# QWTforGithub/CDSegNet

Measured on AMD Instinct MI355X. Metric: points/sec/node (ScanNet ~120k-pt scenes, 1-step), higher is better.
Workload: dtype f16

## Files before the change

### cdsegnet_amd/_lib.py

```python
import ctypes
import os
import threading
from ctypes import POINTER, Structure, c_char_p, c_float, c_int, c_int32, c_int64, c_long, c_size_t, c_uint64, c_void_p

HERE = os.path.dirname(os.path.abspath(__file__))
LIB_PATH = os.path.join(HERE, "libcdseg_hip.so")
LIB_PATH_F16 = os.path.join(HERE, "libcdseg_hip_f16.so")

F32, BF16 = 0, 1
ACT_NONE, ACT_GELU, ACT_SWISH = 0, 1, 2
ORDER_IDS = {"z": 0, "z-trans": 1, "hilbert": 2, "hilbert-trans": 3}
ERRORS = {-1: "CDSEG_ERR_ARG", -2: "CDSEG_ERR_LAUNCH", -3: "CDSEG_ERR_WORKSPACE", -4: "CDSEG_ERR_UNSUPPORTED"}


class CdsegError(RuntimeError):
    pass


class DuplicateVoxelsError(CdsegError):

    def __init__(self, msg, count):
        super().__init__(msg)
        self.count = int(count)

# ... 126 lines not shown
    "cdseg_attn_tail_fused": (c_int, [c_void_p, c_int, c_void_p, c_void_p, c_void_p, c_void_p, c_float, c_void_p, c_void_p,
                                      c_void_p, c_void_p, c_void_p, c_int, c_void_p, c_int, c_long, c_int, c_int, c_void_p]),
    "cdseg_cpe_head_fused": (c_int, [c_void_p, c_int, c_void_p, c_void_p, c_void_p, c_void_p, c_void_p, c_int, c_void_p,
                                     c_void_p, c_void_p, c_float, c_void_p, c_void_p, c_void_p, c_int, c_long, c_int, c_int,
                                     c_int, c_void_p]),
    "cdseg_subm_conv3_wimg_bytes": (c_size_t, [c_int]),
    "cdseg_subm_conv3_pack": (c_int, [c_void_p, c_int, c_void_p, c_void_p]),
    "cdseg_subm_conv3": (c_int, [c_void_p, c_int, c_void_p, c_void_p, c_void_p, c_long, c_int, c_void_p, c_int, c_void_p]),
    "cdseg_child_info": (c_int, [c_void_p, c_void_p, c_long, c_void_p, c_void_p]),
    "cdseg_stem5_wimg_bytes": (c_size_t, []),
    "cdseg_stem5_pack": (c_int, [c_void_p, c_void_p, c_void_p]),
    "cdseg_stem5": (c_int, [c_void_p, c_void_p, c_void_p, c_void_p, c_void_p, c_void_p, c_void_p, c_void_p, c_long, c_long,
                            c_int, c_void_p, c_void_p, c_void_p]),
    "cdseg_block_rr_img_bytes": (c_size_t, [c_int, c_int]),
    "cdseg_block_rr_pack": (c_int, [c_int, c_void_p, c_void_p, c_void_p, c_void_p, c_void_p, c_void_p, c_void_p, c_void_p]),
    "cdseg_cpe_head_rr": (c_int, [c_void_p, c_int, c_void_p, c_void_p, c_void_p, c_void_p, c_void_p, c_int, c_void_p, c_void_p,
                                  c_void_p, c_float, c_void_p, c_void_p, c_int, c_long, c_int, c_int, c_void_p]),
    "cdseg_attn_tail_rr": (c_int, [c_void_p, c_int, c_void_p, c_void_p, c_void_p, c_void_p, c_float, c_void_p, c_void_p,
                                   c_void_p, c_int, c_void_p, c_int, c_long, c_int, c_void_p]),
    "cdseg_cpe_head_rr2": (c_int, [c_void_p, c_int, c_void_p, c_void_p, c_void_p, c_void_p, c_void_p, c_int, c_void_p, c_int,
                                   c_void_p, c_void_p, c_void_p, c_float, c_void_p, c_void_p, c_int, c_long, c_int, c_int, c_void_p]),
    "cdseg_attn_tail_rr2": (c_int, [c_void_p, c_int, c_void_p, c_void_p, c_void_p, c_void_p, c_float, c_void_p, c_void_p,
                                    c_void_p, c_int, c_void_p, c_int, c_void_p, c_int, c_long, c_int, c_void_p, c_size_t, c_void_p]),
    "cdseg_block_scratch_bytes": (c_size_t, [POINTER(BlockDesc), c_long]),
    "cdseg_block_forward": (c_int, [POINTER(BlockDesc), POINTER(BlockIO), c_void_p]),
    "cdseg_layernorm": (c_int, [c_void_p, c_int, c_int, c_void_p, c_void_p, c_float, c_void_p, c_int, c_void_p,
                                c_void_p, c_int, c_int, c_void_p, c_int, c_int, c_long, c_int, c_void_p]),
    "cdseg_attention": (c_int, [c_void_p, c_void_p, c_void_p, c_int, c_int, c_int, c_void_p, c_void_p, c_void_p,
                                c_void_p, c_int, c_int, c_int, c_float, c_void_p, c_int, c_int, c_void_p]),
    "cdseg_attention_ex": (c_int, [c_void_p, c_void_p, c_void_p, c_int, c_int, c_int, c_void_p, c_void_p, c_void_p,
                                   c_void_p, c_int, c_int, c_int, c_float, c_void_p, c_int, c_int, c_int, c_void_p]),
    "cdseg_attention_schedule": (c_long, [c_int, c_int, c_int, c_int, c_void_p, c_long]),
    "cdseg_attention_bwd_ws_bytes": (c_size_t, [c_long, c_int]),
    "cdseg_attention_bwd": (c_int, [c_void_p, c_void_p, c_void_p, c_int, c_int, c_int, c_void_p, c_void_p, c_void_p, c_void_p,
                                    c_int, c_int, c_long, c_int, c_float, c_void_p, c_int, c_void_p, c_void_p, c_void_p,
                                    c_int, c_int, c_int, c_int, c_void_p, c_size_t, c_void_p]),
    "cdseg_layernorm_bwd": (c_int, [c_void_p, c_int, c_void_p, c_float, c_void_p, c_int, c_void_p, c_int, c_int, c_void_p,
                                    c_void_p, c_long, c_int, c_void_p]),
    "cdseg_gelu_bwd": (c_int, [c_void_p, c_void_p, c_void_p, c_long, c_void_p]),
    "cdseg_conv_wgrad": (c_int, [c_void_p, c_int, c_void_p, c_int, c_void_p, c_int, c_long, c_int, c_int, c_void_p, c_void_p,
                                 c_void_p]),
    "cdseg_linear_wgrad": (c_int, [c_void_p, c_int, c_void_p, c_void_p, c_int, c_long, c_int, c_int, c_void_p, c_int, c_void_p,
                                   c_void_p]),
    "cdseg_prof_enable": (c_int, [c_int]),
    "cdseg_prof_summary": (c_int, [POINTER(ctypes.c_double), POINTER(c_long)]),
    "cdseg_prof_summary_class": (c_int, [c_int, POINTER(ctypes.c_double), POINTER(c_long)]),
    "cdseg_segment_max": (c_int, [c_void_p, c_int, c_int, c_void_p, c_long, c_int, c_void_p, c_void_p, c_int,
                                  c_void_p, c_int, c_void_p, c_int, c_int, c_void_p]),
    "cdseg_segment_mean": (c_int, [c_void_p, c_int, c_void_p, c_long, c_int, c_void_p, c_int, c_void_p]),
    "cdseg_pool_fused_img_bytes": (c_size_t, [c_int, c_int]),
    "cdseg_pool_fused_pack": (c_int, [c_void_p, c_int, c_int, c_void_p, c_void_p]),
    "cdseg_pool_fused": (c_int, [c_void_p, c_int, c_void_p, c_void_p, c_void_p, c_long, c_void_p, c_void_p, c_int, c_void_p, c_int,
                                 c_void_p, c_int, c_int, c_int, c_void_p]),
    "cdseg_gemv": (c_int, [c_void_p, c_void_p, c_void_p, c_int, c_int, c_int, c_void_p, c_void_p]),
    "cdseg_randn": (c_int, [c_void_p, c_long, c_uint64, c_uint64, c_void_p]),
    "cdseg_cast": (c_int, [c_void_p, c_int, c_void_p, c_int, c_long, c_void_p]),
    "cdseg_gather_pad_cast": (c_int, [c_void_p, c_int, c_void_p, c_long, c_int, c_int, c_void_p, c_int, c_void_p]),
    "cdseg_ddim_update": (c_int, [c_void_p, c_void_p, c_float, c_float, c_float, c_float, c_int, c_void_p, c_long,
                                  c_void_p]),
    "cdseg_axpy": (c_int, [c_void_p, c_void_p, c_float, c_void_p, c_long, c_void_p]),
    "cdseg_count_saturated": (c_int, [c_void_p, c_long, c_int, c_int, c_void_p, c_void_p]),
    "cdseg_subm_conv3_f32": (c_int, [c_void_p, c_int, c_void_p, c_void_p, c_void_p, c_long, c_int, c_void_p, c_int, c_float, c_int,
                                     c_void_p]),
    "cdseg_split16": (c_int, [c_void_p, c_int, c_long, c_int, c_void_p, c_void_p, c_int, c_float, c_void_p]),
}

_libs = {}
_tls = threading.local()
VARIANTS = ("bf16", "f16")


def active():
    return getattr(_tls, "variant", "bf16")


class use:

    def __init__(self, variant):
        if variant not in VARIANTS:
            raise ValueError(variant)
        self.variant = variant

    def __enter__(self):
        self.prev = active()
        _tls.variant = self.variant
        return self

    def __exit__(self, *exc):
        _tls.variant = self.prev
        return False


def activate(variant):
    if variant not in VARIANTS:
        raise ValueError(variant)
    _tls.variant = variant


def load(variant=None):
    v = variant or active()
    lib = _libs.get(v)
    if lib is not None:
        return lib
    path = LIB_PATH if v == "bf16" else LIB_PATH_F16
    if not os.path.exists(path):
        raise CdsegError(
# ... 15 lines not shown
```

### cdsegnet_amd/csrc/pool.hip

```cpp
#include <atomic>

#include "common.h"

namespace {

struct PoolP {
  const bf16_t* x; const uint4* wimg; const float* bias; const int32_t* seg; const float* scale; const float* shift;
  float* out; bf16_t* out2;
  long m;
  int ldx, ldo, ldo2, act;
};

constexpr int PL_WAVES = 8;

template <int CIN, int COUT>
struct PoolCfg {
  static constexpr int KS = CIN / 32, OT = COUT / 16, QI = CIN / 4, QO = COUT / 4;
  static constexpr int W_BYTES = CIN * COUT * 2;
  static constexpr int ROW = COUT * 2 + 16;
  static constexpr int STRIP = 16 * ROW;
  static constexpr int PAR = 3 * COUT * 4;
  static constexpr int LDS = W_BYTES + PL_WAVES * STRIP + PAR;
};

// ... 102 lines not shown
      float* o = p.out + mrow * p.ldo + q * QO;
#pragma unroll
      for (int c4 = 0; c4 < QO / 4; ++c4) {
        const f32x4_t sc = *reinterpret_cast<const f32x4_t*>(pr + COUT + q * QO + 4 * c4);
        const f32x4_t sh = *reinterpret_cast<const f32x4_t*>(pr + 2 * COUT + q * QO + 4 * c4);
        f32x4_t v;
#pragma unroll
        for (int r = 0; r < 4; ++r) {
          v[r] = __builtin_fmaf(mx[4 * c4 + r], sc[r], sh[r]);
          if (p.act == CDSEG_ACT_GELU) v[r] = gelu_erf(v[r]);
        }
        *reinterpret_cast<f32x4_t*>(o + 4 * c4) = v;
        if (p.out2) {
          uint2 u;
          u.x = pack_bf16x2(v[0], v[1]);
          u.y = pack_bf16x2(v[2], v[3]);
          *reinterpret_cast<uint2*>(p.out2 + mrow * p.ldo2 + q * QO + 4 * c4) = u;
        }
      }
    }
  }
}

__global__ void pool_pack_kernel(const bf16_t* __restrict__ w, uint4* __restrict__ img, int cin, int cout) {
  const int KS = cin / 32;
  const int u = blockIdx.x * blockDim.x + threadIdx.x;
  if (u >= (cout / 16) * KS * 64) return;
  const int lane = u & 63, s = (u >> 6) % KS, ot = (u >> 6) / KS;
  const int q = lane >> 4, i = lane & 15;
  const long row = (i >> 2) * (cout / 4) + ot * 4 + (i & 3);
  img[u] = *reinterpret_cast<const uint4*>(w + row * cin + 32 * s + 8 * q);
}

template <int CIN, int COUT>
int launch_pool(const PoolP& p, hipStream_t s) {
  using K = PoolCfg<CIN, COUT>;
  static std::atomic<bool> attr_done{false};
  if (!attr_done) {
    if (hipFuncSetAttribute((const void*)pool_fused_kernel<CIN, COUT>, hipFuncAttributeMaxDynamicSharedMemorySize, K::LDS) != hipSuccess)
      return CDSEG_ERR_LAUNCH;
    attr_done = true;
  }
  const long chunks = (p.m + 15) / 16;
  long blocks = (chunks + PL_WAVES - 1) / PL_WAVES;
  const int per_cu = K::LDS > 80 * 1024 ? 1 : (K::LDS > 52 * 1024 ? 2 : 3);
  if (blocks > 256 * per_cu) blocks = 256 * per_cu;
  hipLaunchKernelGGL((pool_fused_kernel<CIN, COUT>), dim3((unsigned)blocks), dim3(PL_WAVES * 64), K::LDS, s, p);
  CDSEG_CHECK_LAUNCH();
  return CDSEG_OK;
}

bool pool_supported(int cin, int cout) { return (cin == 32 && cout == 64) || (cin == 64 && cout == 128); }

}

extern "C" size_t cdseg_pool_fused_img_bytes(int cin, int cout) { return pool_supported(cin, cout) ? (size_t)cin * cout * 2 : 0; }

extern "C" int cdseg_pool_fused_pack(const void* w, int cin, int cout, void* wimg, void* stream) {
  if (!w || !wimg || (((uintptr_t)w | (uintptr_t)wimg) & 15)) return CDSEG_ERR_ARG;
  if (!pool_supported(cin, cout)) return CDSEG_ERR_UNSUPPORTED;
  const int units = (cout / 16) * (cin / 32) * 64;
  hipLaunchKernelGGL(pool_pack_kernel, dim3((units + 255) / 256), dim3(256), 0, (hipStream_t)stream, (const bf16_t*)w, (uint4*)wimg, cin,
                     cout);
  CDSEG_CHECK_LAUNCH();
  return CDSEG_OK;
}

extern "C" int cdseg_pool_fused(const void* x, int ldx, const void* wimg, const float* bias, const int32_t* seg_start, long m,
                                const float* scale, const float* shift, int act, float* out, int ldo, void* out2, int ldo2,
                                int cin, int cout, void* stream) {
  if (m <= 0) return CDSEG_OK;
  if (!x || !wimg || !seg_start || !out) return CDSEG_ERR_ARG;
  if (!pool_supported(cin, cout) || (act != CDSEG_ACT_NONE && act != CDSEG_ACT_GELU)) return CDSEG_ERR_UNSUPPORTED;
  if ((ldx & 7) || (ldo & 3) || (out2 && (ldo2 & 3)) || (((uintptr_t)x | (uintptr_t)wimg | (uintptr_t)out) & 15) ||
      (out2 && (((uintptr_t)out2) & 7)) || (bias && (((uintptr_t)bias) & 15)) || (scale && (((uintptr_t)scale) & 15)) ||
      (shift && (((uintptr_t)shift) & 15)) || (!scale != !shift))
    return CDSEG_ERR_ARG;
  PoolP p;
  p.x = (const bf16_t*)x; p.wimg = (const uint4*)wimg; p.bias = bias; p.seg = seg_start; p.scale = scale; p.shift = shift;
  p.out = out; p.out2 = (bf16_t*)out2; p.m = m; p.ldx = ldx; p.ldo = ldo; p.ldo2 = ldo2; p.act = act;
  hipStream_t s = (hipStream_t)stream;
  if (cin == 32) return launch_pool<32, 64>(p, s);
  return launch_pool<64, 128>(p, s);
}
```

### cdsegnet_amd/engine.py

```python
import math
import struct
import os
import threading

import numpy as np
import torch

from . import _lib, ops
from ._lib import CdsegError, DuplicateVoxelsError

CURVES = ("z", "z-trans", "hilbert", "hilbert-trans")


def _pooling_depth(stride):
    return (math.ceil(stride) - 1).bit_length()


class _ShareEvents(threading.local):
    on = False


SHARE_EVENTS = _ShareEvents()


# ... 291 lines not shown

        def bn(mod, pre):
            scale = mod.weight.detach().double() / torch.sqrt(mod.running_var.detach().double() + mod.eps)
            shift = mod.bias.detach().double() - mod.running_mean.detach().double() * scale
            w[pre + ".scale"], w[pre + ".shift"] = f32(scale), f32(shift)

        self.block_desc = {}

        def block(mod, pre):
            self._blocks_to_describe.append((mod, pre))
            conv(mod.cpe[0], pre + ".cpe0")
            lin(mod.cpe[1], pre + ".cpe1")
            ln(mod.cpe[2], pre + ".cpe2")
            ln(mod.norm1[0], pre + ".norm1")
            lin_q(mod.attn.qkv, pre + ".qkv", mod.attn.scale, mod.channels)
            lin(mod.attn.proj, pre + ".proj")
            ln(mod.norm2[0], pre + ".norm2")
            lin(mod.mlp[0].fc1, pre + ".fc1")
            lin(mod.mlp[0].fc2, pre + ".fc2")

        def stem(mod, pre):
            cw = mod.stem.conv.weight.detach()
            cout, cin = cw.shape[0], cw.shape[-1]
            cpad = (cin + 7) // 8 * 8
            wp = torch.zeros(cout, cw.shape[1] ** 3, cpad, dtype=torch.float32)
            wp[:, :, :cin] = cw.reshape(cout, -1, cin).float().cpu()
            w[pre + ".w"] = wp.reshape(cout, -1).to(device=device, dtype=T).contiguous()
            w[pre + ".cpad"] = cpad
            if cw.shape[1] == 5 and cpad == 8 and hasattr(ops, "stem5_pack") and ops.stem5_ok(cout, T):
                w[pre + ".wimg"] = ops.stem5_pack(w[pre + ".w"])
            bn(mod.stem.norm, pre + ".bn")

        def pool(mod, pre):
            lin(mod.proj, pre + ".proj")
            bn(mod.norm[0], pre + ".bn")
            pw = w[pre + ".proj.w"]
            if hasattr(ops, "pool_fused_ok") and ops.pool_fused_ok(pw.shape[1], pw.shape[0], T):
                w[pre + ".proj.wimg"] = ops.pool_fused_pack(pw)

        def unpool(mod, pre):
            lin(mod.proj[0], pre + ".proj")
            bn(mod.proj[1], pre + ".proj_bn")
            lin(mod.proj_skip[0], pre + ".skip")
            bn(mod.proj_skip[1], pre + ".skip_bn")
            if mod.skip_connection_mode == "cat":
                f = (2 ** -0.5 if mod.skip_connection_scale else 1.0)
                if mod.skip_connection_scale_i is not None:
                    f *= 0.8 ** (int(mod.skip_connection_scale_i) - 1)
                wc = mod.proj_cat[0].weight.detach().float()
                c = wc.shape[0]
                w[pre + ".cat_a.w"] = (wc[:, :c] * f).to(device=device, dtype=T).contiguous()
                w[pre + ".cat_b.w"] = wc[:, c:].to(device=device, dtype=T).contiguous()
                w[pre + ".cat.b"] = f32(mod.proj_cat[0].bias)

        bb = self.model.backbone
        stem(bb._n_embedding, "n_emb")
        for s in range(bb.n_num_stages):
            enc = getattr(bb._n_enc, f"enc{s}")
            if s > 0:
                pool(enc.down, f"n_enc{s}.down")
            for name, mod in enc._modules.items():
                if name.startswith("block"):
                    block(mod, f"n_enc{s}.{name}")
        for s in range(bb.n_num_stages - 1):
            dec = getattr(bb._n_dec, f"dec{s}")
            unpool(dec.up, f"n_dec{s}.up")
            for name, mod in dec._modules.items():
                if name.startswith("block"):
                    block(mod, f"n_dec{s}.{name}")
        if isinstance(bb._n_head, torch.nn.Linear):
            lin(bb._n_head, "n_head")
        if bb.condition:
            stem(bb._c_embedding, "c_emb")
            tw, tb, toff = [], [], {}
            off = 0
            for s in range(bb.c_num_stages):
                enc = getattr(bb._c_enc, f"enc{s}")
                if s > 0:
                    pool(enc.down, f"c_enc{s}.down")
                for name, mod in enc._modules.items():
                    if name.startswith("block"):
                        block(mod, f"c_enc{s}.{name}")
                        if bb.T_dim != -1:
                            tw.append(f32(mod.t_mlp.weight))
                            tb.append(f32(mod.t_mlp.bias))
                            toff[f"c_enc{s}.{name}"] = (off, off + mod.channels)
                            off += mod.channels
            for s in range(bb.c_num_stages - 1):
                dec = getattr(bb._c_dec, f"dec{s}")
                unpool(dec.up, f"c_dec{s}.up")
                for name, mod in dec._modules.items():
                    if name.startswith("block"):
                        block(mod, f"c_dec{s}.{name}")
                        if bb.T_dim != -1:
                            tw.append(f32(mod.t_mlp.weight))
                            tb.append(f32(mod.t_mlp.bias))
                            toff[f"c_dec{s}.{name}"] = (off, off + mod.channels)
                            off += mod.channels
            if isinstance(bb._c_head, torch.nn.Linear):
                lin(bb._c_head, "c_head")
            if bb.T_dim != -1:
                w["t.fc1.w"], w["t.fc1.b"] = f32(bb.fc_t1.weight), f32(bb.fc_t1.bias)
                w["t.fc2.w"], w["t.fc2.b"] = f32(bb.fc_t2.weight), f32(bb.fc_t2.bias)
                w["t.mlp.w"], w["t.mlp.b"] = torch.cat(tw).contiguous(), torch.cat(tb).contiguous()
                w["t.table"] = f32(self.model.t_emb_table)
                self.t_slices = toff
# ... 578 lines not shown
            ops.gemm(o, w[pre + ".proj.w"], st.x, bias=w[pre + ".proj.b"], res=st.x)
        self._mlp(st, pre + ".norm2", pre + ".fc", h2)

    def run_embedding(self, plan, feat, perm, pre, curves):
        w, lv = self.w, plan.levels[0]
        cout = w[pre + ".w"].shape[0]
        a = ops.gather_pad_cast(feat, perm, w[pre + ".cpad"], self.T)
        x = self._buf(lv.n, cout, torch.float32)
        xc = x if self.T == torch.float32 else self._buf(lv.n, cout, self.T)
        if (pre + ".wimg") in w and lv.parent is not None and lv.n < (1 << 24):
            par, (cluster, seg) = lv.parent
            ops.stem5(a, w[pre + ".wimg"], w[pre + ".bn.scale"], w[pre + ".bn.shift"], lv.grid, cluster, par.nbr(3, True),
                      lv.child_info(), lv.depth, x, None if xc is x else xc)
        else:
            ops.gemm(a, w[pre + ".w"], x, scale=w[pre + ".bn.scale"], shift=w[pre + ".bn.shift"], act=ops.ACT_GELU,
                     nbr=lv.nbr(5, True), nbr_kmajor=True, kvol=125, out2=None if xc is x else xc)
        self._sat_note(xc)
        return State(lv, x, xc, curves)

    def run_pooling(self, plan, st, pre, cum_to, perm):
        w = self.w
        fine, coarse = st.level, plan.levels[cum_to]
        _, seg = plan.link(fine.cum, cum_to)
        cout = w[pre + ".proj.w"].shape[0]
        x = self._buf(coarse.n, cout, torch.float32)
        xc = x if self.T == torch.float32 else self._buf(coarse.n, cout, self.T)
        if (pre + ".proj.wimg") in w and st.xc.stride(0) == st.xc.shape[1] and fine.n <= 5 * coarse.n:
            ops.pool_fused(st.xc, w[pre + ".proj.wimg"], w[pre + ".proj.b"], seg, coarse.n, w[pre + ".bn.scale"],
                           w[pre + ".bn.shift"], ops.ACT_GELU, x, xc)
        else:
            y = self._buf(fine.n, cout, self.T)
            ops.gemm(st.xc, w[pre + ".proj.w"], y, bias=w[pre + ".proj.b"])
            ops.segment_max(y, seg, coarse.n, w[pre + ".bn.scale"], w[pre + ".bn.shift"], ops.ACT_GELU, x,
                            None if xc is x else xc)
        self._sat_note(xc)
        curves = st.curves if perm is None else [st.curves[int(j)] for j in perm]
        out = State(coarse, x, xc, curves)
        out.parent = st
        return out

    def run_unpooling(self, plan, st, pre, mod):
        w = self.w
        parent = st.parent
        fine, coarse = parent.level, st.level
        cluster, _ = plan.link(fine.cum, coarse.cum)
        cout = w[pre + ".proj.w"].shape[0]
        f = (2 ** -0.5 if mod.skip_connection_scale else 1.0)
        if mod.skip_connection_scale_i is not None:
            f *= 0.8 ** (int(mod.skip_connection_scale_i) - 1)
        x = self._buf(fine.n, cout, torch.float32)
        xc = self._buf(fine.n, cout, self.T)
        if mod.skip_connection_mode == "add":
            assert f == 1.0, "rejected by SerializedUnpooling.__init__"
            child = self._buf(coarse.n, cout, torch.float32)
            ops.gemm(st.xc, w[pre + ".proj.w"], child, bias=w[pre + ".proj.b"], scale=w[pre + ".proj_bn.scale"],
                     shift=w[pre + ".proj_bn.shift"], act=ops.ACT_GELU)
            ops.gemm(parent.xc, w[pre + ".skip.w"], x, bias=w[pre + ".skip.b"], scale=w[pre + ".skip_bn.scale"],
                     shift=w[pre + ".skip_bn.shift"], act=ops.ACT_GELU, add_src=child, add_idx=cluster, out2=xc,
                     out2_pre_add=True)
        else:
            child = self._buf(coarse.n, cout, self.T)
            ops.gemm(st.xc, w[pre + ".proj.w"], child, bias=w[pre + ".proj.b"], scale=w[pre + ".proj_bn.scale"],
                     shift=w[pre + ".proj_bn.shift"], act=ops.ACT_GELU)
            z = self._buf(coarse.n, cout, torch.float32)
            ops.gemm(child, w[pre + ".cat_b.w"], z)
            ops.gemm(parent.xc, w[pre + ".skip.w"], xc, bias=w[pre + ".skip.b"], scale=w[pre + ".skip_bn.scale"],
                     shift=w[pre + ".skip_bn.shift"], act=ops.ACT_GELU)
            ops.gemm(xc, w[pre + ".cat_a.w"], x, bias=w[pre + ".cat.b"], add_src=z, add_idx=cluster)
        self._sat_note(xc)
        out = State(fine, x, xc, parent.curves)
        out.parent = parent.parent
        return out

    def run_cross_block(self, nst, cst):
        w = self.w
        cb = self.model.backbone._tm_dec0.cross_block2
        att = cb.attn
        lv, clv = nst.level, cst.level
        if clv is not lv and list(clv.offs_host) != list(lv.offs_host):
            raise CdsegError("cross attention needs the same number of c- and n-branch bottleneck points per batch "
                             "element (ref: ptv3.py:1009 reuses the q padding for kv)")
        n, cq = nst.x.shape
        self._cpe(nst, "x.q_cpe", nst.xc)
        self._cpe(cst, "x.kv_cpe", cst.xc)
        hq = self._buf(n, cq, self.T)
        ops.layernorm(nst.x, w["x.q_norm1.g"], w["x.q_norm1.b"], hq)
        hkv = self._buf(n, cst.x.shape[1], self.T)
        ops.layernorm(cst.x, w["x.kv_norm1.g"], w["x.kv_norm1.b"], hkv)
        cst.xc = hkv
        if self.T == torch.float32:
            cst.x = hkv
        q = self._buf(n, cq, self.T)
        ops.gemm(hq, w["x.q.w"], q, bias=w["x.q.b"])
        kv = self._buf(n, 2 * cq, self.T)
        ops.gemm(hkv, w["x.kv.w"], kv, bias=w["x.kv.b"])
        K = att.q_patch_size
        q_gidx, widx = lv.slots(nst.curves[att.order_index], K, att.enable_flash)
        kv_gidx, _ = clv.slots(cst.curves[att.order_index], K, att.enable_flash)
        _, _, _, _, patch_start, max_len, sum_l2 = lv.pad(K, att.enable_flash)
        work = 64.0 * att.num_heads * lv.attn_l2(K, att.enable_flash)
        self._add_work(work, 4.0 * n * cq * q.element_size())
        o = self._buf(n, cq, self.T)
        ops.attention(q, kv[:, :cq], kv[:, cq:], q_gidx, kv_gidx, widx, patch_start, att.num_heads, max_len, att.scale, o,
                      work=work, flags=ops.ATTN_Q_PRESCALED if self.q_prescaled else 0)
        if "x.tail_img" in w and n >= ops.DEEP512_MIN_ROWS:
            nst.xc = self._buf(n, cq, self.T)
            ops.attn_tail_rr(o, w["x.tail_img"], w["x.proj.b"], w["x.q_norm2.g"], w["x.q_norm2.b"], w["x.fc1.b"], w["x.fc2.b"],
                             nst.x, nst.xc)
            return
        if "x.tail_img" in w and hasattr(ops, "attn_tail_rr2"):
            x_new = self._buf(n, cq, torch.float32)
            nst.xc = self._buf(n, cq, self.T)
# ... 356 lines not shown
```

### cdsegnet_amd/ops.py

```python
import ctypes
import os
import threading

import torch

from . import _lib
from ._lib import ACT_GELU, ACT_NONE, ACT_SWISH, BF16, F32, GemmArgs, check

__all__ = ["ACT_NONE", "ACT_GELU", "ACT_SWISH", "F32", "BF16"]

LP_DTYPES = {"bf16": torch.bfloat16, "f16": torch.float16}


class _Dtypes:

    def __getitem__(self, dtype):
        if dtype == torch.float32:
            return F32
        if dtype == LP_DTYPES[_lib.active()]:
            return BF16
        raise _lib.CdsegError(f"{dtype} tensors do not belong to the active build of the library ({_lib.active()})")


_DT = _Dtypes()
# ... 743 lines not shown
                                      out2.stride(0) if out2 is not None else 0, m, c, _stream()), "layernorm")
    return out


ATTN_Q_PRESCALED, ATTN_V_BF16 = 1, 2


def attention(q, k, v, q_gidx, kv_gidx, widx, patch_start, num_heads, max_len, scale, out, work=0.0, flags=0):
    num_patches = patch_start.numel() - 1
    if not (q.dtype == k.dtype == out.dtype) or (v.dtype != q.dtype and not (flags & ATTN_V_BF16)):
        raise _lib.CdsegError("attention: q, k, v, out must share a dtype")
    tok = TIMER.begin("attention") if TIMER is not None else None
    check(_lib.load().cdseg_attention_ex(_ptr(q), _ptr(k), _ptr(v), q.stride(0), k.stride(0), v.stride(0), _ptr(q_gidx),
                                         _ptr(kv_gidx), _ptr(widx), _ptr(patch_start), num_patches, int(num_heads),
                                         int(max_len), float(scale), _ptr(out), out.stride(0),
                                         F32X3 if (_TLS.f32x3 and q.dtype == torch.float32) else dt(q), int(flags), _stream()),
          "attention")
    if tok is not None:
        TIMER.end(tok, work)
    return out


def segment_max(y, seg_start, m, scale, shift, act, out, out2=None):
    c = y.shape[1]
    check(_lib.load().cdseg_segment_max(_ptr(y), dt(y), y.stride(0), _ptr(seg_start), m, c, _ptr(scale), _ptr(shift),
                                        int(act), _ptr(out), out.stride(0), _ptr(out2),
                                        dt(out2) if out2 is not None else 0, out2.stride(0) if out2 is not None else 0,
                                        _stream()), "segment_max")
    return out


def pool_fused_ok(cin, cout, dtype):
    return is_lp(dtype) and (int(cin), int(cout)) in ((32, 64), (64, 128))


def pool_fused_pack(w):
    _need_gpu(w)
    cout, cin = w.shape
    lib = _lib.load()
    img = torch.empty(lib.cdseg_pool_fused_img_bytes(cin, cout), dtype=torch.uint8, device=w.device)
    check(lib.cdseg_pool_fused_pack(_ptr(w), cin, cout, _ptr(img), _stream()), "pool_fused_pack")
    return img


def pool_fused(x, wimg, bias, seg_start, m, scale, shift, act, out, out2=None):
    _need_gpu(x, out)
    cin, cout = x.shape[1], out.shape[1]
    check(_lib.load().cdseg_pool_fused(_ptr(x), x.stride(0), _ptr(wimg), _ptr(bias), _ptr(seg_start), int(m), _ptr(scale),
                                       _ptr(shift), int(act), _ptr(out), out.stride(0), _ptr(out2),
                                       out2.stride(0) if out2 is not None else 0, cin, cout, _stream()), "pool_fused")
    return out


def segment_mean(x, seg_start, m):
    out = torch.empty((m, x.shape[1]), dtype=torch.float32, device=x.device)
    check(_lib.load().cdseg_segment_mean(_ptr(x), x.stride(0), _ptr(seg_start), m, x.shape[1], _ptr(out),
                                         out.stride(0), _stream()), "segment_mean")
    return out


def gemv(w, b, x, act=ACT_NONE):
    n, k = w.shape
    y = torch.empty(n, dtype=torch.float32, device=w.device)
    check(_lib.load().cdseg_gemv(_ptr(w), _ptr(b), _ptr(x), n, k, int(act), _ptr(y), _stream()), "gemv")
    return y


def randn(shape, seed, offset, device):
    out = torch.empty(shape, dtype=torch.float32, device=device)
    check(_lib.load().cdseg_randn(_ptr(out), out.numel(), int(seed) & (2 ** 64 - 1), int(offset), _stream()), "randn")
    return out


def cast(src, dtype):
    src = src.contiguous()
    out = torch.empty(src.shape, dtype=dtype, device=src.device)
    check(_lib.load().cdseg_cast(_ptr(src), dt(src), _ptr(out), _DT[dtype], src.numel(), _stream()), "cast")
    return out


def gather_pad_cast(src, idx, cpad, dtype):
    src = src.contiguous()
    n = idx.numel() if idx is not None else src.shape[0]
    out = torch.empty((n, cpad), dtype=dtype, device=src.device)
    check(_lib.load().cdseg_gather_pad_cast(_ptr(src), src.stride(0), _ptr(idx), n, src.shape[1], int(cpad), _ptr(out),
                                            _DT[dtype], _stream()), "gather_pad_cast")
    return out


def ddim_update(xt, eps, sqrt_ab_prev, sqrt_1m_ab, sqrt_ab, sqrt_1m_ab_prev, final=False):
    out = torch.empty_like(xt)
    check(_lib.load().cdseg_ddim_update(_ptr(xt), _ptr(eps), float(sqrt_ab_prev), float(sqrt_1m_ab), float(sqrt_ab),
                                 float(sqrt_1m_ab_prev), 1 if final else 0, _ptr(out), xt.numel(), _stream()),
          "ddim_update")
    return out


def axpy(a, b, alpha):
    out = torch.empty_like(a)
    check(_lib.load().cdseg_axpy(_ptr(a), _ptr(b), float(alpha), _ptr(out), a.numel(), _stream()), "axpy")
    return out


def voxelize(coord, grid_size):
    _need_gpu(coord)
    coord = coord.float().contiguous()
# ... 218 lines not shown
```

### include/cdseg.h

```cpp
#ifndef CDSEG_H
#define CDSEG_H

#include <stddef.h>
#include <stdint.h>

#ifdef __cplusplus
extern "C" {
#endif

#define CDSEG_OK 0
#define CDSEG_ERR_ARG (-1)
#define CDSEG_ERR_LAUNCH (-2)
#define CDSEG_ERR_WORKSPACE (-3)
#define CDSEG_ERR_UNSUPPORTED (-4)

#define CDSEG_F32 0
#define CDSEG_BF16 1
#define CDSEG_F32X3 2

#define CDSEG_ORDER_Z 0
#define CDSEG_ORDER_Z_TRANS 1
#define CDSEG_ORDER_HILBERT 2
#define CDSEG_ORDER_HILBERT_TRANS 3

// ... 75 lines not shown
  const int32_t* out_idx;
  void* out;
  void* out2;
  long M;
  int N, K, kvol;
  int lda, ldo, ldo2, ldres, ldadd;
  int a_dtype, compute_dtype, out_dtype, out2_dtype;
  int act;
  int out2_pre_add;
  void* ws;
  size_t ws_bytes;
  const float* colbias;
  const float* ln_pre_g;
  const float* ln_pre_b;
  const float* ln_post_g;
  const float* ln_post_b;
  void* ln_out;
  int ldln, ln_out_dtype;
  float ln_eps;
  int nbr_kmajor;
} cdseg_gemm_args;
int cdseg_gemm(const cdseg_gemm_args* args_host, void* stream);

int cdseg_layernorm(const void* x, int x_dtype, int ldx, const float* gamma, const float* beta, float eps,
                    const float* res, int ldres, const float* colbias, void* out, int out_dtype, int ldo,
                    void* out2, int out2_dtype, int ldo2, long m, int c, void* stream);

int cdseg_attention(const void* q, const void* k, const void* v, int ldq, int ldk, int ldv, const int32_t* q_gidx,
                    const int32_t* kv_gidx, const int32_t* widx, const int32_t* patch_start, int num_patches,
                    int num_heads, int max_len, float scale, void* out, int ldo, int dtype, void* stream);
#define CDSEG_ATTN_Q_PRESCALED 1
#define CDSEG_ATTN_V_BF16 2
int cdseg_attention_ex(const void* q, const void* k, const void* v, int ldq, int ldk, int ldv, const int32_t* q_gidx,
                       const int32_t* kv_gidx, const int32_t* widx, const int32_t* patch_start, int num_patches,
                       int num_heads, int max_len, float scale, void* out, int ldo, int dtype, int flags, void* stream);

long cdseg_attention_schedule(int num_patches, int num_heads, int max_len, int dtype, int32_t* table, long capacity);

int cdseg_prof_enable(int on);
int cdseg_prof_summary(double* total_ms, long* launches);
#define CDSEG_PROF_ATTENTION 0
#define CDSEG_PROF_CONV 1
#define CDSEG_PROF_CONV_DEEP 2
int cdseg_prof_summary_class(int cls, double* total_ms, long* launches);

int cdseg_segment_max(const void* y, int y_dtype, int ldy, const int32_t* seg_start, long m, int c,
                      const float* scale, const float* shift, int act, float* out, int ldo, void* out2,
                      int out2_dtype, int ldo2, void* stream);
size_t cdseg_pool_fused_img_bytes(int cin, int cout);
int cdseg_pool_fused_pack(const void* w, int cin, int cout, void* wimg, void* stream);
int cdseg_pool_fused(const void* x, int ldx, const void* wimg, const float* bias, const int32_t* seg_start, long m,
                     const float* scale, const float* shift, int act, float* out, int ldo, void* out2, int ldo2,
                     int cin, int cout, void* stream);
int cdseg_segment_mean(const float* x, int ldx, const int32_t* seg_start, long m, int c, float* out, int ldo,
                       void* stream);

int cdseg_gemv(const float* w, const float* b, const float* x, int n, int k, int act, float* y, void* stream);
int cdseg_randn(float* out, long n, uint64_t seed, uint64_t offset, void* stream);
int cdseg_cast(const void* src, int src_dtype, void* dst, int dst_dtype, long n, void* stream);
int cdseg_gather_pad_cast(const float* src, int ld_src, const int32_t* idx, long n, int cin, int cpad, void* dst,
                          int dst_dtype, void* stream);
int cdseg_ddim_update(const float* xt, const float* eps, float sqrt_ab_prev, float sqrt_1m_ab, float sqrt_ab,
                      float sqrt_1m_ab_prev, int final_step, float* out, long n, void* stream);
int cdseg_count_saturated(const void* x, long rows, int cols, int ld, unsigned long long* counter, void* stream);
int cdseg_subm_conv3_f32(const void* x, int ldx, const void* wimg, const float* bias, const int32_t* nbr_kmajor, long n,
                         int channels, float* yf, int ldyf, float out_scale, int accumulate, void* stream);
int cdseg_split16(const float* x, int ldx, long rows, int cols, void* hi, void* lo, int ld16, float lo_scale, void* stream);
int cdseg_axpy(const float* a, const float* b, float alpha, float* out, long n, void* stream);

int cdseg_voxelize(const float* coord, double grid_size, long n, int32_t* grid, int64_t* key, int32_t* min3_dev,
                   void* stream);
int cdseg_voxelize_f64(const double* coord, double grid_size, long n, int32_t* grid, int64_t* key, int32_t* min3_dev,
                       void* stream);
int cdseg_center_shift(const void* xyz, int is_f64, long n, int apply_z, void* out, void* ws12, void* stream);
int cdseg_tta_apply(const float* in, long n, const double* rot9_host, double scale, int apply_scale, int flip, void* out,
                    void* stream);
int cdseg_div_add(const float* in, float div, float add, long n, float* out, void* stream);
int cdseg_collect_feat(const float* a, int ca, const void* b, int b_is_f64, int cb, long n, float* out, void* stream);
int cdseg_max_run(const int32_t* seg_start, long m, int32_t* out_dev, void* stream);
int cdseg_fragment_select(const int32_t* idx_sort, const int32_t* seg_start, long m, int frag, int32_t* idx_part,
                          void* stream);
int cdseg_softmax_vote(const float* logits, int ldl, const int32_t* idx, long m, int c, float* pred, int ldp,
                       void* stream);
int cdseg_argmax_rows(const float* x, int ldx, long n, int c, int32_t* out, void* stream);

int cdseg_knn(const float* ref_xyz, const int32_t* ref_offset, long n, const float* qry_xyz, const int32_t* qry_offset,
              long m, int nb, int k, const float* origin, float cell, int32_t* idx, float* dist2, void* ws, size_t ws_bytes,
              void* stream);
size_t cdseg_knn1_ws_bytes(long n);
int cdseg_knn1(const float* ref_xyz, const int32_t* ref_offset, long n, const float* qry_xyz, const int32_t* qry_offset,
               long m, int nb, const float* origin, float cell, int32_t* idx, float* dist2, void* ws, size_t ws_bytes,
               void* stream);
int cdseg_iou_counts(const int32_t* pred, const int32_t* pred_idx, const int32_t* target, long n, int k, int ignore_index,
                     int64_t* out, void* stream);

int cdseg_mlp_fused(const void* h, int ldh, const void* w1, const float* b1, const void* w2, const float* b2, float* x,
                    int ldx, void* xc, int ldxc, long n, int channels, int dtype, void* stream);

int cdseg_attn_tail_fused(const void* o, int ldo, const void* wp, const float* bp, const float* ln_g, const float* ln_b,
                          float ln_eps, const void* w1, const float* b1, const void* w2, const float* b2, float* x, int ldx,
                          void* xc, int ldxc, long n, int channels, int dtype, void* stream);

int cdseg_cpe_head_fused(const void* y, int ldy, const void* wl, const float* bl, const float* lnp_g, const float* lnp_b,
                         float* x, int ldx, const float* colbias, const float* ln1_g, const float* ln1_b, float eps,
                         const void* wqkv, const float* bqkv, void* qkv, int ldqkv, long n, int channels, int dtype,
                         int qkv_flags, void* stream);
// ... 160 lines not shown
```

Before: 80.27 million.

## Fuse unpooling skip and projection GEMMs with gather into one kernel

Adds a fused unpool kernel that computes, per fine row, both the skip linear on the fine features and the projection linear on the gathered coarse parent features. Each branch gets bias, BN scale/shift and GELU, then the sum is written in f32 alongside the pre-add low-precision copy. It is used for the 'add' skip mode when the channel configuration is supported. This replaces two GEMM launches and the intermediate f32 child buffer. In exchange, the projection is recomputed once per fine point rather than once per coarse point.

```diff
diff --git a/cdsegnet_amd/_lib.py b/cdsegnet_amd/_lib.py
--- a/cdsegnet_amd/_lib.py
+++ b/cdsegnet_amd/_lib.py
@@ -202,6 +202,11 @@
     "cdseg_pool_fused_pack": (c_int, [c_void_p, c_int, c_int, c_void_p, c_void_p]),
     "cdseg_pool_fused": (c_int, [c_void_p, c_int, c_void_p, c_void_p, c_void_p, c_long, c_void_p, c_void_p, c_int, c_void_p, c_int,
                                  c_void_p, c_int, c_int, c_int, c_void_p]),
+    "cdseg_unpool_fused_img_bytes": (c_size_t, [c_int, c_int, c_int]),
+    "cdseg_unpool_fused_sweep_rows": (c_long, []),
+    "cdseg_unpool_fused_pack": (c_int, [c_void_p, c_void_p, c_int, c_int, c_int, c_void_p, c_void_p]),
+    "cdseg_unpool_fused": (c_int, [c_void_p, c_int, c_void_p, c_int, c_void_p, c_long, c_void_p, c_void_p, c_void_p, c_void_p,
+                                   c_void_p, c_void_p, c_void_p, c_void_p, c_int, c_void_p, c_int, c_int, c_int, c_int, c_void_p]),
     "cdseg_gemv": (c_int, [c_void_p, c_void_p, c_void_p, c_int, c_int, c_int, c_void_p, c_void_p]),
     "cdseg_randn": (c_int, [c_void_p, c_long, c_uint64, c_uint64, c_void_p]),
     "cdseg_cast": (c_int, [c_void_p, c_int, c_void_p, c_int, c_long, c_void_p]),
diff --git a/cdsegnet_amd/csrc/pool.hip b/cdsegnet_amd/csrc/pool.hip
--- a/cdsegnet_amd/csrc/pool.hip
+++ b/cdsegnet_amd/csrc/pool.hip
@@ -178,6 +178,117 @@
 
 bool pool_supported(int cin, int cout) { return (cin == 32 && cout == 64) || (cin == 64 && cout == 128); }
 
+struct UnpoolP {
+  const bf16_t* skip; const bf16_t* coarse; const int32_t* cluster; const uint4* wimg;
+  const float* par[6];
+  float* x; bf16_t* xc;
+  long n;
+  int lds, ldc, ldx, ldxc;
+};
+
+constexpr int UP_WAVES = 8;
+constexpr int UP_MAX_BLOCKS = 1024;
+
+template <int CS, int CC, int COUT>
+__global__ __launch_bounds__(UP_WAVES * 64) void unpool_fused_kernel(UnpoolP p) {
+  constexpr int KSS = CS / 32, KSC = CC / 32, OT = COUT / 16, QO = COUT / 4;
+  constexpr int WS_BYTES = CS * COUT * 2, W_BYTES = (CS + CC) * COUT * 2;
+  __shared__ __attribute__((aligned(16))) char smem[W_BYTES + 6 * COUT * 4];
+  const int tid = threadIdx.x, lane = tid & 63;
+  const int wave = __builtin_amdgcn_readfirstlane(tid >> 6);
+  const int j = lane & 15, q = lane >> 4;
+  {
+    uint4* d = reinterpret_cast<uint4*>(smem);
+    for (int u = tid; u < W_BYTES / 16; u += UP_WAVES * 64) d[u] = p.wimg[u];
+    float* pr = reinterpret_cast<float*>(smem + W_BYTES);
+#pragma unroll
+    for (int v = 0; v < 6; ++v)
+      for (int c = tid; c < COUT; c += UP_WAVES * 64) pr[v * COUT + c] = p.par[v][c];
+  }
+  __syncthreads();
+  const uint4* Ws = reinterpret_cast<const uint4*>(smem);
+  const uint4* Wp = reinterpret_cast<const uint4*>(smem + WS_BYTES);
+  const float* pr = reinterpret_cast<const float*>(smem + W_BYTES) + q * QO;
+
+  const long groups = (p.n + 15) / 16;
+  const long stride = (long)gridDim.x * UP_WAVES;
+  long g = (long)blockIdx.x * UP_WAVES + wave;
+  if (g >= groups) return;
+  auto row_of = [&](long gg) {
+    const long r = gg * 16 + j;
+    return r < p.n ? r : p.n - 1;
+  };
+  auto fetch_skip = [&](long r, bf16x8_t (&dst)[KSS]) {
+#pragma unroll
+    for (int s = 0; s < KSS; ++s) dst[s] = *reinterpret_cast<const bf16x8_t*>(p.skip + r * p.lds + 32 * s + 8 * q);
+  };
+  auto fetch_coarse = [&](int c, bf16x8_t (&dst)[KSC]) {
+#pragma unroll
+    for (int s = 0; s < KSC; ++s) dst[s] = *reinterpret_cast<const bf16x8_t*>(p.coarse + (long)c * p.ldc + 32 * s + 8 * q);
+  };
+  bf16x8_t xs[KSS], xq[KSC];
+  fetch_skip(row_of(g), xs);
+  fetch_coarse(p.cluster[row_of(g)], xq);
+  long gn = g + stride;
+  int cnext = p.cluster[row_of(gn < groups ? gn : g)];
+#pragma unroll 1
+  for (; g < groups; g = gn, gn += stride) {
+    const long g1 = gn < groups ? gn : g, g2 = gn + stride < groups ? gn + stride : g1;
+    bf16x8_t xsn[KSS], xqn[KSC];
+    fetch_skip(row_of(g1), xsn);
+    fetch_coarse(cnext, xqn);
+    cnext = p.cluster[row_of(g2)];
+    int lo = lane;
+    asm volatile("" : "+v"(lo));
+    const long row = g * 16 + j;
+    const bool valid = row < p.n;
+    float* xo = p.x + row * p.ldx + q * QO;
+    uint4 u;
+#pragma unroll
+    for (int t = 0; t < OT; ++t) {
+      f32x4_t a = {0.f, 0.f, 0.f, 0.f}, c = {0.f, 0.f, 0.f, 0.f};
+#pragma unroll
+      for (int s = 0; s < KSS; ++s) a = mfma_16x16x32_bf16(__builtin_bit_cast(bf16x8_t, Ws[(t * KSS + s) * 64 + lo]), xs[s], a);
+#pragma unroll
+      for (int s = 0; s < KSC; ++s) c = mfma_16x16x32_bf16(__builtin_bit_cast(bf16x8_t, Wp[(t * KSC + s) * 64 + lo]), xq[s], c);
+      a += *reinterpret_cast<const f32x4_t*>(pr + 4 * t);
+      c += *reinterpret_cast<const f32x4_t*>(pr + 3 * COUT + 4 * t);
+      const f32x4_t sa = *reinterpret_cast<const f32x4_t*>(pr + COUT + 4 * t), ha = *reinterpret_cast<const f32x4_t*>(pr + 2 * COUT + 4 * t);
+      const f32x4_t sc = *reinterpret_cast<const f32x4_t*>(pr + 4 * COUT + 4 * t), hc = *reinterpret_cast<const f32x4_t*>(pr + 5 * COUT + 4 * t);
+      f32x4_t v;
+#pragma unroll
+      for (int r = 0; r < 4; ++r) {
+        a[r] = gelu_erf(__builtin_fmaf(a[r], sa[r], ha[r]));
+        c[r] = gelu_erf(__builtin_fmaf(c[r], sc[r], hc[r]));
+        v[r] = a[r] + c[r];
+      }
+      if (valid) *reinterpret_cast<f32x4_t*>(xo + 4 * t) = v;
+      if (t & 1) {
+        u.z = pack_bf16x2(a[0], a[1]); u.w = pack_bf16x2(a[2], a[3]);
+        if (valid && p.xc) *reinterpret_cast<uint4*>(p.xc + row * p.ldxc + q * QO + 4 * (t - 1)) = u;
+      } else {
+        u.x = pack_bf16x2(a[0], a[1]); u.y = pack_bf16x2(a[2], a[3]);
+      }
+    }
+#pragma unroll
+    for (int s = 0; s < KSS; ++s) xs[s] = xsn[s];
+#pragma unroll
+    for (int s = 0; s < KSC; ++s) xq[s] = xqn[s];
+  }
+}
+
+template <int CS, int CC, int COUT>
+int launch_unpool(const UnpoolP& p, hipStream_t s) {
+  const long groups = (p.n + 15) / 16;
+  long blocks = (groups + UP_WAVES - 1) / UP_WAVES;
+  if (blocks > UP_MAX_BLOCKS) blocks = UP_MAX_BLOCKS;
+  hipLaunchKernelGGL((unpool_fused_kernel<CS, CC, COUT>), dim3((unsigned)blocks), dim3(UP_WAVES * 64), 0, s, p);
+  CDSEG_CHECK_LAUNCH();
+  return CDSEG_OK;
+}
+
+bool unpool_supported(int cs, int cc, int cout) { return cout == 64 && ((cs == 32 && cc == 64) || (cs == 64 && cc == 128)); }
+
 }
 
 extern "C" size_t cdseg_pool_fused_img_bytes(int cin, int cout) { return pool_supported(cin, cout) ? (size_t)cin * cout * 2 : 0; }
@@ -209,3 +320,43 @@
   if (cin == 32) return launch_pool<32, 64>(p, s);
   return launch_pool<64, 128>(p, s);
 }
+
+extern "C" size_t cdseg_unpool_fused_img_bytes(int cs, int cc, int cout) {
+  return unpool_supported(cs, cc, cout) ? (size_t)(cs + cc) * cout * 2 : 0;
+}
+
+extern "C" long cdseg_unpool_fused_sweep_rows(void) { return (long)UP_MAX_BLOCKS * UP_WAVES * 16; }
+
+extern "C" int cdseg_unpool_fused_pack(const void* w_skip, const void* w_proj, int cs, int cc, int cout, void* wimg, void* stream) {
+  if (!w_skip || !w_proj || !wimg || (((uintptr_t)w_skip | (uintptr_t)w_proj | (uintptr_t)wimg) & 15)) return CDSEG_ERR_ARG;
+  if (!unpool_supported(cs, cc, cout)) return CDSEG_ERR_UNSUPPORTED;
+  const int us = (cout / 16) * (cs / 32) * 64, up = (cout / 16) * (cc / 32) * 64;
+  hipLaunchKernelGGL(pool_pack_kernel, dim3((us + 255) / 256), dim3(256), 0, (hipStream_t)stream, (const bf16_t*)w_skip, (uint4*)wimg, cs,
+                     cout);
+  CDSEG_CHECK_LAUNCH();
+  hipLaunchKernelGGL(pool_pack_kernel, dim3((up + 255) / 256), dim3(256), 0, (hipStream_t)stream, (const bf16_t*)w_proj, (uint4*)wimg + us,
+                     cc, cout);
+  CDSEG_CHECK_LAUNCH();
+  return CDSEG_OK;
+}
+
+extern "C" int cdseg_unpool_fused(const void* skip, int ld_skip, const void* coarse, int ld_coarse, const int32_t* cluster, long n,
+                                  const void* wimg, const float* bias_s, const float* scale_s, const float* shift_s,
+                                  const float* bias_p, const float* scale_p, const float* shift_p, float* x, int ldx, void* xc,
+                                  int ldxc, int cs, int cc, int cout, void* stream) {
+  if (n <= 0) return CDSEG_OK;
+  if (!unpool_supported(cs, cc, cout)) return CDSEG_ERR_UNSUPPORTED;
+  if (!skip || !coarse || !cluster || !wimg || !bias_s || !scale_s || !shift_s || !bias_p || !scale_p || !shift_p || !x)
+    return CDSEG_ERR_ARG;
+  if (ld_skip < cs || ld_coarse < cc || ldx < cout || (xc && ldxc < cout) || (ld_skip & 7) || (ld_coarse & 7) || (ldx & 3) ||
+      (xc && (ldxc & 7)) || (((uintptr_t)skip | (uintptr_t)coarse | (uintptr_t)wimg | (uintptr_t)x | (uintptr_t)xc) & 15) ||
+      ((uintptr_t)cluster & 3))
+    return CDSEG_ERR_ARG;
+  UnpoolP p;
+  p.skip = (const bf16_t*)skip; p.coarse = (const bf16_t*)coarse; p.cluster = cluster; p.wimg = (const uint4*)wimg;
+  p.par[0] = bias_s; p.par[1] = scale_s; p.par[2] = shift_s; p.par[3] = bias_p; p.par[4] = scale_p; p.par[5] = shift_p;
+  p.x = x; p.xc = (bf16_t*)xc; p.n = n; p.lds = ld_skip; p.ldc = ld_coarse; p.ldx = ldx; p.ldxc = ldxc;
+  hipStream_t s = (hipStream_t)stream;
+  if (cs == 32) return launch_unpool<32, 64, 64>(p, s);
+  return launch_unpool<64, 128, 64>(p, s);
+}
diff --git a/cdsegnet_amd/engine.py b/cdsegnet_amd/engine.py
--- a/cdsegnet_amd/engine.py
+++ b/cdsegnet_amd/engine.py
@@ -367,6 +367,11 @@
                 w[pre + ".cat_a.w"] = (wc[:, :c] * f).to(device=device, dtype=T).contiguous()
                 w[pre + ".cat_b.w"] = wc[:, c:].to(device=device, dtype=T).contiguous()
                 w[pre + ".cat.b"] = f32(mod.proj_cat[0].bias)
+            elif hasattr(ops, "unpool_fused_ok"):
+                ws, wp = w[pre + ".skip.w"], w[pre + ".proj.w"]
+                if ops.unpool_fused_ok(ws.shape[1], wp.shape[1], ws.shape[0], T) and all(
+                        w.get(pre + k) is not None for k in (".skip.b", ".proj.b")):
+                    w[pre + ".wimg"] = ops.unpool_fused_pack(ws, wp)
 
         bb = self.model.backbone
         stem(bb._n_embedding, "n_emb")
@@ -1051,12 +1056,17 @@
         xc = self._buf(fine.n, cout, self.T)
         if mod.skip_connection_mode == "add":
             assert f == 1.0, "rejected by SerializedUnpooling.__init__"
-            child = self._buf(coarse.n, cout, torch.float32)
-            ops.gemm(st.xc, w[pre + ".proj.w"], child, bias=w[pre + ".proj.b"], scale=w[pre + ".proj_bn.scale"],
-                     shift=w[pre + ".proj_bn.shift"], act=ops.ACT_GELU)
-            ops.gemm(parent.xc, w[pre + ".skip.w"], x, bias=w[pre + ".skip.b"], scale=w[pre + ".skip_bn.scale"],
-                     shift=w[pre + ".skip_bn.shift"], act=ops.ACT_GELU, add_src=child, add_idx=cluster, out2=xc,
-                     out2_pre_add=True)
+            if w.get(pre + ".wimg") is not None:
+                ops.unpool_fused(parent.xc, st.xc, cluster, w[pre + ".wimg"],
+                                 (w[pre + ".skip.b"], w[pre + ".skip_bn.scale"], w[pre + ".skip_bn.shift"]),
+                                 (w[pre + ".proj.b"], w[pre + ".proj_bn.scale"], w[pre + ".proj_bn.shift"]), x, xc)
+            else:
+                child = self._buf(coarse.n, cout, torch.float32)
+                ops.gemm(st.xc, w[pre + ".proj.w"], child, bias=w[pre + ".proj.b"], scale=w[pre + ".proj_bn.scale"],
+                         shift=w[pre + ".proj_bn.shift"], act=ops.ACT_GELU)
+                ops.gemm(parent.xc, w[pre + ".skip.w"], x, bias=w[pre + ".skip.b"], scale=w[pre + ".skip_bn.scale"],
+                         shift=w[pre + ".skip_bn.shift"], act=ops.ACT_GELU, add_src=child, add_idx=cluster, out2=xc,
+                         out2_pre_add=True)
         else:
             child = self._buf(coarse.n, cout, self.T)
             ops.gemm(st.xc, w[pre + ".proj.w"], child, bias=w[pre + ".proj.b"], scale=w[pre + ".proj_bn.scale"],
diff --git a/cdsegnet_amd/ops.py b/cdsegnet_amd/ops.py
--- a/cdsegnet_amd/ops.py
+++ b/cdsegnet_amd/ops.py
@@ -819,6 +819,33 @@
     return out
 
 
+def unpool_fused_ok(cs, cc, cout, dtype):
+    return is_lp(dtype) and (int(cs), int(cc), int(cout)) in ((32, 64, 64), (64, 128, 64))
+
+
+def unpool_fused_sweep_rows():
+    return int(_lib.load().cdseg_unpool_fused_sweep_rows())
+
+
+def unpool_fused_pack(w_skip, w_proj):
+    _need_gpu(w_skip, w_proj)
+    (cout, cs), cc = w_skip.shape, w_proj.shape[1]
+    lib = _lib.load()
+    img = torch.empty(lib.cdseg_unpool_fused_img_bytes(cs, cc, cout), dtype=torch.uint8, device=w_skip.device)
+    check(lib.cdseg_unpool_fused_pack(_ptr(w_skip), _ptr(w_proj), cs, cc, cout, _ptr(img), _stream()), "unpool_fused_pack")
+    return img
+
+
+def unpool_fused(skip, coarse, cluster, wimg, skip_bss, proj_bss, x, xc=None):
+    _need_gpu(skip, coarse, x)
+    check(_lib.load().cdseg_unpool_fused(_ptr(skip), skip.stride(0), _ptr(coarse), coarse.stride(0), _ptr(cluster), skip.shape[0],
+                                         _ptr(wimg), _ptr(skip_bss[0]), _ptr(skip_bss[1]), _ptr(skip_bss[2]), _ptr(proj_bss[0]),
+                                         _ptr(proj_bss[1]), _ptr(proj_bss[2]), _ptr(x), x.stride(0), _ptr(xc),
+                                         xc.stride(0) if xc is not None else 0, skip.shape[1], coarse.shape[1], x.shape[1],
+                                         _stream()), "unpool_fused")
+    return x
+
+
 def segment_mean(x, seg_start, m):
     out = torch.empty((m, x.shape[1]), dtype=torch.float32, device=x.device)
     check(_lib.load().cdseg_segment_mean(_ptr(x), x.stride(0), _ptr(seg_start), m, x.shape[1], _ptr(out),
diff --git a/include/cdseg.h b/include/cdseg.h
--- a/include/cdseg.h
+++ b/include/cdseg.h
@@ -151,6 +151,13 @@
 int cdseg_pool_fused(const void* x, int ldx, const void* wimg, const float* bias, const int32_t* seg_start, long m,
                      const float* scale, const float* shift, int act, float* out, int ldo, void* out2, int ldo2,
                      int cin, int cout, void* stream);
+size_t cdseg_unpool_fused_img_bytes(int cs, int cc, int cout);
+long cdseg_unpool_fused_sweep_rows(void);
+int cdseg_unpool_fused_pack(const void* w_skip, const void* w_proj, int cs, int cc, int cout, void* wimg, void* stream);
+int cdseg_unpool_fused(const void* skip, int ld_skip, const void* coarse, int ld_coarse, const int32_t* cluster, long n,
+                       const void* wimg, const float* bias_s, const float* scale_s, const float* shift_s,
+                       const float* bias_p, const float* scale_p, const float* shift_p, float* x, int ldx, void* xc,
+                       int ldxc, int cs, int cc, int cout, void* stream);
 int cdseg_segment_mean(const float* x, int ldx, const int32_t* seg_start, long m, int c, float* out, int ldo,
                        void* stream);
 
```

Result: no change. 80.94 million, median of 6 (+0.8%).
